# Orbiter-Finance/Plonky2-lib

Measured on AMD Instinct MI355X. Metric: proofs/sec for secp256k1 ECDSA-verify circuit; Goldilocks NTT GB/s vs HBM peak, higher is better.
Workload: dtype u64 (Goldilocks, 64-bit modular integer)

## Files before the change

### plonky2-lib_amd/csrc/circuit_create.inc

```

static int build_quotient_plan(glp_ctx *c, glp_circuit *cc) {
    const glp_circuit_desc &d = cc->d;
    std::vector<u64> desc((size_t)LIMB_GROUPS * d.num_wires * LIMB_SLOTS, 0);
    for (int g = 0; g < LIMB_GROUPS; g++) { cc->limb_jlo[g] = d.num_wires; cc->limb_jhi[g] = 0; }
    auto put = [&](u32 s, u32 col, u32 pos, u32 kl, bool flush, u32 kf, u32 ref) {
        const u32 grp = s / LIMB_SLOTS, slot = s % LIMB_SLOTS;
        desc[((size_t)grp * d.num_wires + col) * LIMB_SLOTS + slot] = 1ull | ((u64)pos << 1) | (flush ? 32ull : 0ull) | ((u64)kl << 6) | ((u64)kf << 16) | ((u64)ref << 26);
        cc->limb_jlo[grp] = std::min(cc->limb_jlo[grp], col); cc->limb_jhi[grp] = std::max(cc->limb_jhi[grp], col);
    };
    std::vector<GateShape> shape(d.num_gates);
    for (u32 gi = 0; gi < d.num_gates; gi++) gate_shape(cc->gates[gi], shape[gi]);
    std::vector<u32> limb_list;
    auto fill = [&](u32 s, u32 gi) {
        const LimbBlock &b = shape[gi].limb;
        cc->limb_gi[s] = gi;
        for (u32 i = 0; i < b.ops; i++)
            for (u32 j = 0; j < b.limbs; j++)
                put(s, b.first + b.limbs * i + j, j & 15, b.kstride * i + b.klimb + (b.descending ? b.limbs - 1 - j : j), (j & 15) == 15 || j + 1 == b.limbs,
                    b.kstride * i + b.ksum + (j >> 4), b.ref_stride * i + b.ref0 + (j >> 4));
    };
    auto limb_start = [&](u32 gi) -> u32 { return shape[gi].limb.first; };
    auto limb_weight = [&](u32 gi) -> u32 { return shape[gi].limb.limbs * shape[gi].limb.ops; };
    for (u32 gi = 0; gi < d.num_gates; gi++) {
        const glp_gate &g = cc->gates[gi];
// ... 6 lines not shown
        } else if (light && cc->light_count < 8) {
            cc->light_gi[cc->light_count++] = gi;
        } else if (g.type != GLP_GATE_NOOP) {
            cc->single_gates.push_back(gi);
        }
    }
    if (limb_list.size() == 1) {
        cc->single_gates.push_back(limb_list[0]);
        limb_list.clear();
    }
    if (!limb_list.empty()) {
        const u32 cnt = (u32)limb_list.size();
        const u32 G = (cnt + LIMB_SLOTS - 1) / LIMB_SLOTS;
        u32 used[LIMB_GROUPS] = {0, 0, 0, 0};
        std::stable_sort(limb_list.begin(), limb_list.end(), [&](u32 x, u32 y) {
            return limb_start(x) != limb_start(y) ? limb_start(x) < limb_start(y) : limb_weight(x) > limb_weight(y); });
        for (u32 t = 0; t < cnt; t++) {
            const u32 grp = t / LIMB_SLOTS;
            fill(grp * LIMB_SLOTS + used[grp], limb_list[t]);
            used[grp]++;
        }
        cc->limb_count = cnt; cc->limb_groups = G;
        for (u32 g = 0; g < G; g++) cc->limb_gcount[g] = used[g];
    }
    if (cc->limb_count) {
        std::vector<u32> keep;
        for (u32 gi : cc->single_gates) {
            if (cc->gates[gi].type == GLP_GATE_COMPARISON && cc->limb_extra_count < 4) cc->limb_extra_gi[cc->limb_extra_count++] = gi;
            else keep.push_back(gi);
        }
        cc->single_gates.swap(keep);
    }
    if (cc->limb_count) {
        GLP_TRY(c->alloc((void **)&cc->dev_limb_desc, desc.size() * 8));
        GLP_TRY(h2d(c, cc->dev_limb_desc, desc.data(), desc.size() * 8));
    }
    return GLP_OK;
}

extern "C" {

void glp_circuit_free(glp_circuit *cc) {
    if (!cc) return;
    glp_ctx *c = cc->ctx;
    (void)hipSetDevice(c->device);
    (void)hipStreamSynchronize(c->stream);
// ... 159 lines not shown
```

### plonky2-lib_amd/csrc/prover.hip

```cpp
#include <algorithm>
#include <string.h>
#include "batch.h"
#include "common.h"
#include "merkle.h"
#include "ntt.h"
#include "poseidon.h"
#include "prover_types.h"

namespace {
void make_layout(const glp_circuit_desc &c, Layout &L, bool zk) {
    const u32 cap = 1u << c.cap_height, nch = c.num_challenges;
    memset(&L, 0, sizeof(L));
    L.oracle_cols[0] = c.num_constants + c.num_routed_wires;
    L.oracle_cols[1] = c.num_wires;
    L.oracle_cols[2] = nch * (1 + c.num_partial_products);
    L.oracle_cols[3] = nch * c.quotient_degree_factor;
    for (int k = 0; k < 4; k++) L.leaf_len[k] = L.oracle_cols[k] + (zk && k > 0 ? SALT_SIZE : 0);
    L.nopen = (size_t)c.num_constants + c.num_routed_wires + c.num_wires + 2 * nch + nch * c.num_partial_products +
              nch * c.quotient_degree_factor;
    L.openings = 3 * (size_t)cap * 4;
    L.fri_caps = L.openings + 2 * L.nopen;
    L.queries = L.fri_caps + (size_t)c.num_reductions * cap * 4;
    const u32 lgN = c.degree_bits + c.rate_bits;
    L.depth0 = lgN - c.cap_height;
// ... 118 lines not shown
        GLP_TRY(commit(dev_wires, BATCH_VALUES, g.nw, wb, GLP_SALT_TAG_WIRES, 0, host_wires));
        stage = S_WIRES;
        return GLP_OK;
    }
    int partial_products(const u64 *betas_in, const u64 *gammas_in) {
        GLP_REQUIRE(stage == S_WIRES, "partial_products: call after begin");
        for (u32 i = 0; i < g.nch; i++) { betas[i] = betas_in[i]; gammas[i] = gammas_in[i]; }
        u64 *zp, *dens, *tot;
        GLP_TRY(tmp.get(&zp, (size_t)g.nzp * g.n));
        GLP_TRY(tmp.get(&dens, (size_t)g.nzp * g.n));
        GLP_TRY(tmp.get(&tot, (size_t)g.nch * nblk(g.n)));
        {
            StageScope st(c, "partial_products", 8.0 * g.n * (2.0 * g.nr + g.nzp));
            GLP_TRY(stage_partial_products(c, g, dev_wires, betas, gammas, nullptr, zp, dens, tot));
        }
        GLP_TRY(commit(zp, BATCH_VALUES, g.nzp, zb, GLP_SALT_TAG_ZS, 1));
        stage = S_ZS;
        return GLP_OK;
    }
    int quotient(const u64 *alphas) {
        GLP_REQUIRE(stage == S_ZS, "quotient: call after partial_products");
        const u32 nch = g.nch;
        const size_t apn = (size_t)nch * g.nterms, qlen = (size_t)nch * g.Rq * g.n;
        std::vector<u64> apow((1 + APL_WORDS) * apn);
        alpha_power_table(alphas, nch, g.nterms, apow.data(), apow.data() + apn);
        u64 *dev_apow, *qv, *qV, *qc;
        GLP_TRY(tmp.get(&dev_apow, apow.size()));
        GLP_TRY(h2d(c, dev_apow, apow.data(), apow.size() * 8));
        GLP_TRY(tmp.get(&qv, qlen));
        GLP_TRY(tmp.get(&qV, qlen));
        GLP_TRY(tmp.get(&qc, qlen));
        QProof qp;
        QBatch qbt;
        quotient_proof_args(g, wb.b, zb.b, qv, dev_apow, nullptr, qp, qbt);
        for (u32 i = 0; i < nch; i++) { qp.betas[i] = betas[i]; qp.gammas[i] = gammas[i]; }
        memcpy(qp.pih, pih, 32);
        {
            StageScope st(c, "quotient_eval", 8.0 * g.n * g.Rq * (g.nc + g.nr + g.nw + g.nzp + 2.0 * nch));
            u64 *l0t;
            GLP_TRY(tmp.get(&l0t, (size_t)g.Rq * g.n));
            GLP_TRY(stage_quotient_eval(c, g, qp, qbt, l0t));
        }
        {
            StageScope st(c, "quotient_intt", 16.0 * g.n * g.Rq * nch);
            GLP_TRY(stage_quotient_coeffs(c, g, qv, qV, qc));
        }
        GLP_TRY(commit(qc, BATCH_COEFFS_BITREV, nch * g.qdf, qb, GLP_SALT_TAG_QUOTIENT, 2));
        stage = S_QUOTIENT;
// ... 371 lines not shown
```

### plonky2-lib_amd/csrc/prover_batch.inc

```
#include "host_pool.h"

namespace {

int caps_to_host(glp_ctx *c, const u64 *dev_digests, size_t dig_stride_words, size_t cap_off_digests, u32 capn, u32 K, std::vector<u64> &out) {
    out.resize((size_t)K * capn * 4);
    GLP_HIP(hipMemcpy2DAsync(out.data(), (size_t)capn * 32, dev_digests + 4 * cap_off_digests, dig_stride_words * 8, (size_t)capn * 32, K,
                             hipMemcpyDeviceToHost, c->stream));
    GLP_HIP(hipStreamSynchronize(c->stream));
    return GLP_OK;
}

int prove_batch_impl(glp_ctx *c, const glp_circuit *cc, u32 K, const u64 *dev_wires, const u64 *public_inputs, u64 *proofs_out) {
    const glp_circuit_desc &d = cc->d;
    const Layout &L = cc->L;
    const ProveGeo g = prove_geo(cc, K);
    GLP_TRY(batch_check(g));
    const int lg = g.lg, rb = g.rb, hasher = g.hasher;
    const size_t n = g.n, N = g.N;
    const u32 nch = g.nch, nw = g.nw, qdf = g.qdf, nzp = g.nzp, capn = g.capn, nterms = g.nterms, npi = d.num_public_inputs;
    const u32 nred = d.num_reductions, nq = d.num_query_rounds;
    HostPool &pool = ctx_host_pool(c);
    BatchTrace mark(c, K, "");
    Tmp tmp(c);
    auto P = [&](u32 k) { return proofs_out + (size_t)k * L.total; };
// ... 16 lines not shown
    std::vector<u64> chal((size_t)K * 2 * MAXCH, 0);
    pool.run(K, [&](size_t k) {
        memcpy(P((u32)k) + L.caps, &caps[k * capn * 4], (size_t)capn * 32);
        ch[k].observe_hashes(cc->digest, 1);
        ch[k].observe(&pih[4 * k], 4);
        ch[k].observe_hashes(&caps[k * capn * 4], capn);
        for (u32 i = 0; i < nch; i++) chal[k * 2 * MAXCH + i] = ch[k].get();
        for (u32 i = 0; i < nch; i++) chal[k * 2 * MAXCH + MAXCH + i] = ch[k].get();
    });

    mark("transcript 1 (host)");
    u64 *dev_chal, *zp, *dens, *tot;
    GLP_TRY(tmp.get(&dev_chal, chal.size()));
    GLP_TRY(h2d(c, dev_chal, chal.data(), chal.size() * 8));
    GLP_TRY(tmp.get(&zp, (size_t)K * nzp * n));
    GLP_TRY(tmp.get(&dens, (size_t)K * nzp * n));
    GLP_TRY(tmp.get(&tot, (size_t)K * nch * nblk(n)));
    GLP_TRY(stage_partial_products(c, g, dev_wires, nullptr, nullptr, dev_chal, zp, dens, tot));
    GLP_TRY(batch_build(c, zp, BATCH_VALUES, nzp, lg, rb, (int)d.cap_height, &zb.b, nullptr, K, hasher, salt, GLP_SALT_TAG_ZS));
    GLP_TRY(caps_to_host(c, zb.b->digests, ndig * 4, cap_off, capn, K, caps));

    mark("partial products + commit");
    const size_t apn = (size_t)nch * nterms;
    std::vector<u64> apow((size_t)(1 + APL_WORDS) * K * apn), qpp((size_t)K * 3 * MAXCH, 0);
    pool.run(K, [&](size_t k) {
        memcpy(P((u32)k) + L.caps + capn * 4, &caps[k * capn * 4], (size_t)capn * 32);
        ch[k].observe_hashes(&caps[k * capn * 4], capn);
        u64 alphas[MAXCH];
        for (u32 i = 0; i < nch; i++) alphas[i] = ch[k].get();
        alpha_power_table(alphas, nch, nterms, &apow[k * apn], &apow[(size_t)K * apn + APL_WORDS * k * apn]);
        for (u32 i = 0; i < nch; i++) { qpp[k * 3 * MAXCH + i] = chal[k * 2 * MAXCH + i]; qpp[k * 3 * MAXCH + MAXCH + i] = chal[k * 2 * MAXCH + MAXCH + i]; }
        memcpy(&qpp[k * 3 * MAXCH + 2 * MAXCH], &pih[4 * k], 32);
    });
    mark("transcript 2 + alpha powers (host)");
    u64 *dev_apow, *dev_qpp, *qv, *qV, *qc, *l0t;
    GLP_TRY(tmp.get(&dev_apow, apow.size()));
    GLP_TRY(h2d(c, dev_apow, apow.data(), apow.size() * 8));
    GLP_TRY(tmp.get(&dev_qpp, qpp.size()));
    GLP_TRY(h2d(c, dev_qpp, qpp.data(), qpp.size() * 8));
    const size_t qstride = (size_t)nch * g.Rq * n;
    GLP_TRY(tmp.get(&qv, (size_t)K * qstride));
    GLP_TRY(tmp.get(&qV, (size_t)K * qstride));
    GLP_TRY(tmp.get(&qc, (size_t)K * qstride));
    GLP_TRY(tmp.get(&l0t, (size_t)g.Rq * n));
    {
        QProof qp;
        QBatch qbt;
        quotient_proof_args(g, wb.b, zb.b, qv, dev_apow, dev_qpp, qp, qbt);
        GLP_TRY(stage_quotient_eval(c, g, qp, qbt, l0t));
        GLP_TRY(stage_quotient_coeffs(c, g, qv, qV, qc));
    }
    GLP_TRY(batch_build(c, qc, BATCH_COEFFS_BITREV, nch * qdf, lg, rb, (int)d.cap_height, &qb.b, nullptr, K, hasher, salt, GLP_SALT_TAG_QUOTIENT));
    GLP_TRY(caps_to_host(c, qb.b->digests, ndig * 4, cap_off, capn, K, caps));
// ... 143 lines not shown
```

### plonky2-lib_amd/csrc/prover_batch_dev.inc

```
#include "transcript_dev.h"
namespace {

int prove_batch_impl_dev(glp_ctx *c, const glp_circuit *cc, u32 K, const u64 *dev_wires, const u64 *public_inputs, u64 *proofs_out) {
    const glp_circuit_desc &d = cc->d;
    const Layout &L = cc->L;
    const ProveGeo pg = prove_geo(cc, K);
    GLP_TRY(batch_check(pg));
    const int lg = pg.lg, rb = pg.rb, hasher = pg.hasher;
    const size_t n = pg.n, N = pg.N;
    const u32 nch = pg.nch, nw = pg.nw, qdf = pg.qdf, npp = pg.npp, nzp = pg.nzp, capn = pg.capn, nterms = pg.nterms, npi = d.num_public_inputs;
    const u32 nred = d.num_reductions, nq = d.num_query_rounds;
    BatchTrace mark(c, K, " dev");
    Tmp tmp(c);
    BatchHolder wb, zb, qb;
    u64 salt_seed[4] = {0, 0, 0, 0};
    const u64 *salt = nullptr;
    if (cc->zk) { GLP_TRY(salt_seed_draw(c, salt_seed)); salt = salt_seed; }
    const unsigned tgrid = (K + 15) / 16;
    u64 *dch, *image;
    u32 *dev_err;
    GLP_TRY(tmp.get(&dch, (size_t)K * DCH_WORDS));
    GLP_TRY(tmp.get(&image, (size_t)K * L.total));
    { u64 *e; GLP_TRY(tmp.get(&e, (K + 1) / 2 + 1)); dev_err = (u32 *)e; }
    GLP_HIP(hipMemsetAsync(dev_err, 0, (size_t)K * 4, c->stream));
// ... 1 lines not shown
    TrGeo g;
    g.dch = dch; g.image = image; g.total = L.total; g.K = K; g.capn = capn; g.nch = nch;

    GLP_TRY(batch_build(c, dev_wires, BATCH_VALUES, nw, lg, rb, (int)d.cap_height, &wb.b, nullptr, K, hasher, salt, GLP_SALT_TAG_WIRES));
    const size_t ndig = wb.b->ndigests, cap_off = merkle_cap_offset(N, (int)d.cap_height);
    u64 *dev_chal, *dev_qpp;
    GLP_TRY(tmp.get(&dev_chal, (size_t)K * 2 * MAXCH));
    GLP_TRY(tmp.get(&dev_qpp, (size_t)K * 3 * MAXCH));
    GLP_HIP(hipMemsetAsync(dev_chal, 0, (size_t)K * 2 * MAXCH * 8, c->stream));
    GLP_HIP(hipMemsetAsync(dev_qpp, 0, (size_t)K * 3 * MAXCH * 8, c->stream));
    hipLaunchKernelGGL(k_tr_begin, dim3(tgrid), dim3(256), 0, c->stream, g, cc->digest[0], cc->digest[1], cc->digest[2], cc->digest[3], L.pis, npi,
                       wb.b->digests + 4 * cap_off, ndig * 4, L.caps, dev_chal, dev_qpp);
    GLP_HIP(hipGetLastError());
    mark("wires commit + transcript 1");

    u64 *zp, *dens, *tot;
    GLP_TRY(tmp.get(&zp, (size_t)K * nzp * n));
    GLP_TRY(tmp.get(&dens, (size_t)K * nzp * n));
    GLP_TRY(tmp.get(&tot, (size_t)K * nch * nblk(n)));
    GLP_TRY(stage_partial_products(c, pg, dev_wires, nullptr, nullptr, dev_chal, zp, dens, tot));
    GLP_TRY(batch_build(c, zp, BATCH_VALUES, nzp, lg, rb, (int)d.cap_height, &zb.b, nullptr, K, hasher, salt, GLP_SALT_TAG_ZS));
    const size_t apn = (size_t)nch * nterms;
    u64 *dev_apow, *qv, *qV, *qc, *l0t;
    GLP_TRY(tmp.get(&dev_apow, (size_t)(1 + APL_WORDS) * K * apn));
    hipLaunchKernelGGL(k_tr_alphas, dim3(tgrid), dim3(256), 0, c->stream, g, zb.b->digests + 4 * cap_off, ndig * 4, L.caps + (size_t)capn * 4, nterms, dev_apow,
                       dev_apow + (size_t)K * apn);
    GLP_HIP(hipGetLastError());
    mark("partial products + commit + transcript 2");

    const size_t qstride = (size_t)nch * pg.Rq * n;
    GLP_TRY(tmp.get(&qv, (size_t)K * qstride));
    GLP_TRY(tmp.get(&qV, (size_t)K * qstride));
    GLP_TRY(tmp.get(&qc, (size_t)K * qstride));
    GLP_TRY(tmp.get(&l0t, (size_t)pg.Rq * n));
    {
        QProof qp;
        QBatch qbt;
        quotient_proof_args(pg, wb.b, zb.b, qv, dev_apow, dev_qpp, qp, qbt);
        GLP_TRY(stage_quotient_eval(c, pg, qp, qbt, l0t));
        GLP_TRY(stage_quotient_coeffs(c, pg, qv, qV, qc));
    }
    GLP_TRY(batch_build(c, qc, BATCH_COEFFS_BITREV, nch * qdf, lg, rb, (int)d.cap_height, &qb.b, nullptr, K, hasher, salt, GLP_SALT_TAG_QUOTIENT));
    const u64 wn = root_of_unity(lg);
    u64 *dev_zetas;
    GLP_TRY(tmp.get(&dev_zetas, (size_t)K * 4));
    hipLaunchKernelGGL(k_tr_zeta, dim3(tgrid), dim3(256), 0, c->stream, g, qb.b->digests + 4 * cap_off, ndig * 4, L.caps + 2 * (size_t)capn * 4, (u32)lg, wn, dev_zetas,
                       dev_err);
    GLP_HIP(hipGetLastError());
    mark("quotient + commit + transcript 3");
// ... 97 lines not shown
```

### plonky2-lib_amd/csrc/prover_stages.inc

```
#include <stdlib.h>
#include <chrono>

namespace {

struct ProveGeo {
    const glp_circuit *cc;
    int lg, rb, qdb, hasher, cap_height;
    size_t n, N;
    u32 nch, nr, nw, nc, qdf, npp, nzp, capn, Rq, step, nterms, K;
    const u32 *arity_bits;
    u32 nq;
};
ProveGeo prove_geo(const glp_circuit *cc, u32 K) {
    const glp_circuit_desc &d = cc->d;
    ProveGeo g;
    g.cc = cc; g.K = K;
    g.lg = (int)d.degree_bits; g.rb = (int)d.rate_bits; g.hasher = (int)d.hasher; g.cap_height = (int)d.cap_height;
    g.n = (size_t)1 << g.lg; g.N = g.n << g.rb;
    g.nch = d.num_challenges; g.nr = d.num_routed_wires; g.nw = d.num_wires; g.nc = d.num_constants;
    g.qdf = d.quotient_degree_factor; g.npp = d.num_partial_products;
    g.nzp = g.nch * (1 + g.npp); g.capn = 1u << d.cap_height;
    g.qdb = 0;
    while ((1u << g.qdb) < g.qdf) g.qdb++;
    g.Rq = 1u << g.qdb; g.step = 1u << (g.rb - g.qdb);
// ... 13 lines not shown
    for (u32 i = 0; i < MAXCH; i++) { a.betas[i] = !chal && i < nch ? betas[i] : 0; a.gammas[i] = !chal && i < nch ? gammas[i] : 0; }
    a.w_n = root_of_unity(g.lg); a.lg = lg; a.nr = g.nr; a.nch = nch; a.npp = npp; a.qdf = g.qdf;
    a.chal = chal; a.wires_stride = (size_t)g.nw * g.n; a.zp_stride = (size_t)g.nzp * g.n;
    const size_t small_lds = (size_t)2 * nch * (npp + 2) * g.n * sizeof(u64);
    if (g.lg <= 7 && small_lds <= 64 * 1024) {
        hipLaunchKernelGGL(k_pp_rows_small, dim3(1, K), dim3(256), small_lds, c->stream, a);
        GLP_HIP(hipGetLastError());
        return GLP_OK;
    }
    switch (nch) {
    case 1: hipLaunchKernelGGL(HIP_KERNEL_NAME(k_pp_rows<1>), dim3(nblocks, K), dim3(256), 0, c->stream, a); break;
    case 2: hipLaunchKernelGGL(HIP_KERNEL_NAME(k_pp_rows<2>), dim3(nblocks, K), dim3(256), 0, c->stream, a); break;
    case 3: hipLaunchKernelGGL(HIP_KERNEL_NAME(k_pp_rows<3>), dim3(nblocks, K), dim3(256), 0, c->stream, a); break;
    default: hipLaunchKernelGGL(HIP_KERNEL_NAME(k_pp_rows<4>), dim3(nblocks, K), dim3(256), 0, c->stream, a); break;
    }
    GLP_HIP(hipGetLastError());
    hipLaunchKernelGGL(k_pp_block_tot, dim3(nblocks, nch, K), dim3(256), 0, c->stream, zp, tot, lg, nblocks, a.zp_stride);
    hipLaunchKernelGGL(k_pp_scan_tot, dim3(nch, K), dim3(256), 0, c->stream, tot, nblocks);
    hipLaunchKernelGGL(k_pp_apply, dim3(nblocks, nch, K), dim3(256), 0, c->stream, zp, tot, lg, nblocks, nch, npp, a.zp_stride);
    GLP_HIP(hipGetLastError());
    return GLP_OK;
}

void alpha_power_table(const u64 *alphas, u32 nch, u32 nterms, u64 *whole, u64 *limbs) {
    for (u32 i = 0; i < nch; i++) {
        u64 x = 1;
        for (u32 t = 0; t < nterms; t++) {
            const size_t e = (size_t)i * nterms + t;
            whole[e] = x;
            apl_words(x, limbs + APL_WORDS * e);
            x = mul(x, alphas[i]);
        }
    }
}
void quotient_proof_args(const ProveGeo &g, const glp_batch *wb, const glp_batch *zb, u64 *qv, const u64 *dev_apow, const u64 *dev_pp,
                         QProof &qp, QBatch &qb) {
    memset(&qp, 0, sizeof(qp));
    qb.apow_stride = (size_t)g.nch * g.nterms;
    qp.wl = wb->lde; qp.zl = zb->lde; qp.out = qv; qp.apow = dev_apow; qp.apl = dev_apow + g.K * qb.apow_stride;
    qb.pp = dev_pp; qb.wl_stride = (size_t)(g.nw + wb->salt) * g.N; qb.zl_stride = (size_t)(g.nzp + zb->salt) * g.N;
    qb.out_stride = (size_t)g.nch * g.Rq * g.n;
}
int stage_quotient_eval(glp_ctx *c, const ProveGeo &g, const QProof &qp, const QBatch &qbt, u64 *l0t) {
    const glp_circuit *cc = g.cc;
    const glp_circuit_desc &d = cc->d;
    const u32 nch = g.nch;
    QArgs a;
    a.cs = cc->cs->lde; a.gates = cc->dev_gates; a.k_is = cc->dev_k_is; a.k_ratio = cc->k_ratio;
    const u64 WN = root_of_unity(g.lg + g.rb), gn = pow(GEN, (u64)g.n), wR = root_of_unity(g.rb);
    for (u32 rq = 0; rq < g.Rq; rq++) {
        const u32 r = rq * g.step;
        a.shift_r[rq] = mul(GEN, pow(WN, (u64)r));
        a.zh[rq] = sub(mul(gn, pow(wR, (u64)r)), 1);
        a.zh_inv[rq] = inv(a.zh[rq]);
    }
    a.w_n = root_of_unity(g.lg); a.n_field = (u64)g.n % P;
    a.lg = (u32)g.lg; a.rb = (u32)g.rb; a.step = g.step; a.nc = g.nc; a.nsel = d.num_selectors; a.nr = g.nr; a.nw = g.nw;
    a.nch = nch; a.npp = g.npp; a.qdf = g.qdf; a.num_gates = d.num_gates; a.nterms = g.nterms;
    a.many_selectors = d.num_selectors > 1;
    a.gate_mode = nch == 2 ? 1 : 0;
    a.l0 = l0t;
    hipLaunchKernelGGL(k_l0_table, dim3(nblk(g.n)), dim3(256), 0, c->stream, a, l0t, g.Rq);
    GLP_HIP(hipGetLastError());
    LightArgs lg_;
    lg_.count = cc->light_count; lg_.arith_gi = cc->arith_gi; lg_.arith_ops = cc->arith_ops;
    for (u32 i = 0; i < 8; i++) lg_.gi[i] = cc->light_gi[i];
    const dim3 grid(nblk(g.n), g.Rq, g.K);
    switch (nch) {
    case 1: hipLaunchKernelGGL(HIP_KERNEL_NAME(k_quotient<1, 1>), grid, dim3(256), 0, c->stream, a, qp, qbt, lg_); break;
    case 2:
        if (cc->light_count || cc->arith_ops) hipLaunchKernelGGL(HIP_KERNEL_NAME(k_quotient<2, 2>), grid, dim3(256), 0, c->stream, a, qp, qbt, lg_);
        else hipLaunchKernelGGL(HIP_KERNEL_NAME(k_quotient<2, 0>), grid, dim3(256), 0, c->stream, a, qp, qbt, lg_);
        break;
    case 3: hipLaunchKernelGGL(HIP_KERNEL_NAME(k_quotient<3, 1>), grid, dim3(256), 0, c->stream, a, qp, qbt, lg_); break;
    default: hipLaunchKernelGGL(HIP_KERNEL_NAME(k_quotient<4, 1>), grid, dim3(256), 0, c->stream, a, qp, qbt, lg_); break;
    }
    GLP_HIP(hipGetLastError());
    if (a.gate_mode != 1) return GLP_OK;
    if (cc->limb_count) {
        LimbArgs la;
        limb_args(cc, la);
        la.extra_count = cc->limb_extra_count;
// ... 186 lines not shown
        shift_bits += ly.ab;
        hipLaunchKernelGGL(k_fri_gather_leaf, dim3(nblk((size_t)g.nq * arity), g.K), dim3(256), 0, c->stream, ly.vals, ly.lgL, (u32)g.rb, ly.ab, dev_idx,
                           shift_bits, g.nq, dev_q + off, stride, 2 * Lsz, qsec);
        GLP_HIP(hipGetLastError());
        off += 2 * (size_t)arity;
        GLP_TRY(merkle_gather_paths(c, ly.dig, nleaves, g.cap_height, dev_idx, g.nq, dev_q + off, stride, shift_bits, g.K, ly.ndig * 4, qsec));
        off += 4 * (size_t)(ly.lgL - ly.ab - g.cap_height);
    }
    return GLP_OK;
}
int stage_queries(glp_ctx *c, const ProveGeo &g, const glp_batch *const ob[4], const std::vector<FriLayer> &layers, const u64 *dev_idx,
                  u64 *dev_q, size_t stride, size_t qsec) {
    size_t off = 0;
    for (int b = 0; b < 4; b++) GLP_TRY(queries_oracle(c, g, ob[b], b == 0, dev_idx, dev_q, stride, qsec, off));
    GLP_TRY(queries_layers(c, g, layers, dev_idx, dev_q, stride, qsec, off));
    if (off != stride) return set_error(GLP_ERR_ARG, "internal: query record layout mismatch");
    return GLP_OK;
}

int batch_check(const ProveGeo &g) {
    GLP_REQUIRE(g.nch == 2, "glp_prove_batch: num_challenges = %u (the batch path evaluates the quotient with the two-challenge kernels)", g.nch);
    GLP_REQUIRE(g.K >= 1 && g.K <= 4096, "glp_prove_batch: batch of %u proofs outside 1..4096", g.K);
    GLP_REQUIRE((size_t)g.K * g.nw * g.N * 8 <= ((size_t)64 << 30), "glp_prove_batch: batch too large (K * num_wires * 2^(degree_bits + rate_bits) words)");
    return GLP_OK;
}
struct BatchTrace {
    glp_ctx *c;
    u32 K;
    const char *tag;
    const bool on = getenv("GLP_BATCH_TRACE") != nullptr;
    std::chrono::steady_clock::time_point t_last = std::chrono::steady_clock::now();
    BatchTrace(glp_ctx *ctx, u32 K_, const char *tag_) : c(ctx), K(K_), tag(tag_) {}
    void operator()(const char *what) {
        if (!on) return;
        (void)hipStreamSynchronize(c->stream);
        const auto now = std::chrono::steady_clock::now();
        fprintf(stderr, "[glp_prove_batch K=%u%s] %-28s %8.3f ms\n", K, tag, what, std::chrono::duration<double, std::milli>(now - t_last).count());
        t_last = now;
    }
};

}
```

### plonky2-lib_amd/csrc/quotient_kernels.inc

```
__device__ __forceinline__ u64 range_product(u64 v, u32 bound) {
    if (bound == 4) {
        const u64 u = mul_nc(v, add_cnc(v, P - 3));
        return mul_nc(u, add_cnc(2, u));
    }
    u64 p = v;
    for (u32 x = 1; x + 1 < bound; x++) p = mul(p, sub(v, (u64)x));
    return bound > 1 ? mul_nc(p, sub(v, (u64)(bound - 1))) : p;
}
struct Base4Sum { u64 lo, hi; };
__device__ __forceinline__ void b4_zero(Base4Sum &b) { b.lo = 0; b.hi = 0; }
__device__ __forceinline__ void b4_add(Base4Sum &b, u64 limb, u32 j ) {
    const u32 w = 1u << (2 * j);
    b.lo += (u64)(u32)limb * w;
    b.hi += (u64)(u32)(limb >> 32) * w;
}
__device__ __forceinline__ u64 b4_value(const Base4Sum &b) {
    const u64 l = b.lo + (b.hi << 32);
    const u32 h = (u32)(b.hi >> 32) + (l < b.lo ? 1u : 0u);
    return canon(fold96_nc(l, h));
}
struct Acc160 { u32 w0, w1, w2, w3, w4; };
__device__ __forceinline__ void acc_zero(Acc160 &a) { a.w0 = a.w1 = a.w2 = a.w3 = a.w4 = 0; }
__device__ __forceinline__ void acc_fma(Acc160 &a, u64 v, u64 m) {
    const u32 v0 = (u32)v, v1 = (u32)(v >> 32), m0 = (u32)m, m1 = (u32)(m >> 32);
// ... 38 lines not shown
}
__device__ __forceinline__ u64 acc2_reduce(const AccLimb &a) {
    Acc160 w;
    acc_zero(w);
    acc_add_shifted<0>(w, a.a00); acc_add_shifted<22>(w, a.a10); acc_add_shifted<32>(w, a.a01);
    acc_add_shifted<44>(w, a.a20); acc_add_shifted<54>(w, a.a11); acc_add_shifted<76>(w, a.a21);
    return acc_reduce(w);
}

struct AccHL { u64 c0, c1, c2; };
constexpr u32 ACC3_MAX_TERMS = 512;
inline void apl_words(u64 m, u64 out[4]) {
    const u64 mp = glf::mul(m, 1ull << 32);
    out[0] = (m & 0x3FFFFFull) | (((m >> 22) & 0x3FFFFFull) << 32); out[1] = m >> 44;
    out[2] = (mp & 0x3FFFFFull) | (((mp >> 22) & 0x3FFFFFull) << 32); out[3] = mp >> 44;
}
__device__ __forceinline__ void acc3_zero(AccHL &a) { a.c0 = a.c1 = a.c2 = 0; }
__device__ __forceinline__ void acc3_fma(AccHL &a, u64 v, const u64 *ml) {
    const u32 vlo = (u32)v, vhi = (u32)(v >> 32);
    const u64 w0 = ml[0], w1 = ml[1], w2 = ml[2], w3 = ml[3];
    a.c0 += (u64)vlo * (u32)w0; a.c1 += (u64)vlo * (u32)(w0 >> 32); a.c2 += (u64)vlo * (u32)w1;
    a.c0 += (u64)vhi * (u32)w2; a.c1 += (u64)vhi * (u32)(w2 >> 32); a.c2 += (u64)vhi * (u32)w3;
}
__device__ __forceinline__ u64 acc3_reduce(const AccHL &a) {
    Acc160 w;
    acc_zero(w);
    acc_add_shifted<0>(w, a.c0); acc_add_shifted<22>(w, a.c1); acc_add_shifted<44>(w, a.c2);
    return acc_reduce(w);
}

struct QArgs {
    const u64 *cs;
    const DevGate *gates;
    const u64 *k_is;
    u64 shift_r[MAXR], zh[MAXR], zh_inv[MAXR];
    u64 w_n, n_field;
    u32 lg, rb, step, nc, nsel, nr, nw, nch, npp, qdf, num_gates, nterms, many_selectors, gate_mode;
    u32 k_ratio;
    const u64 *l0;
};
struct QProof {
    const u64 *wl, *zl;
    u64 *out;
    const u64 *apow;
    const u64 *apl;
    u64 betas[MAXCH], gammas[MAXCH], pih[4];
};
struct QBatch { const u64 *pp; size_t wl_stride, zl_stride, out_stride, apow_stride; };
static_assert(MAXCH == 4, "pp layout: 4 betas, 4 gammas, 4 words of the public-input hash");
__device__ __forceinline__ QProof q_proof(const QProof &p0, const QBatch &b) {
    QProof p = p0;
    if (b.pp) {
        const size_t k = blockIdx.z;
        p.wl += k * b.wl_stride; p.zl += k * b.zl_stride; p.out += k * b.out_stride; p.apow += k * b.apow_stride; p.apl += APL_WORDS * k * b.apow_stride;
        const u64 *q = b.pp + k * 3 * MAXCH;
        _Pragma("unroll") for (int c = 0; c < MAXCH; c++) { p.betas[c] = q[c]; p.gammas[c] = q[MAXCH + c]; p.pih[c] = q[2 * MAXCH + c]; }
    }
    return p;
}
__global__ __launch_bounds__(256) void k_l0_table(QArgs a, u64 *out, u32 Rq) {
    const size_t n = (size_t)1 << a.lg;
    const size_t q = (size_t)blockIdx.x * 256 + threadIdx.x;
    if (q >= n) return;
    const u64 wq = dpow(a.w_n, q);
    u64 d[MAXR], pre[MAXR];
    u64 run = 1;
    for (u32 rq = 0; rq < Rq; rq++) {
        d[rq] = mul(a.n_field, sub(mul(a.shift_r[rq], wq), 1));
        pre[rq] = run;
        run = mul(run, d[rq]);
    }
    u64 iv = inv(run);
    for (int rq = (int)Rq - 1; rq >= 0; rq--) {
        out[(size_t)rq * n + q] = mul(a.zh[rq], mul(iv, pre[rq]));
        iv = mul(iv, d[rq]);
    }
}
// ... 505 lines not shown
    const u32 rq = blockIdx.y, r = rq * a.step;
    const size_t slot = (size_t)r * n + q;
    u64 acc[MAXCH];
    _Pragma("unroll") for (int c = 0; c < NCH; c++) acc[c] = 0;
    const DevGate g = a.gates[gi];
    gate_contrib<NCH, TYPE>(a, p, g, N, slot, (u32)NCH + (u32)NCH * (a.npp + 1), acc);
    const size_t Rq = (size_t)gridDim.y;
    _Pragma("unroll") for (int c = 0; c < NCH; c++) {
        u64 *o = p.out + ((size_t)c * Rq + rq) * n + q;
        *o = add(*o, mul(acc[c], a.zh_inv[rq]));
    }
}

constexpr int LIMB_SLOTS = 5, LIMB_GROUPS = 4;
struct LimbArgs { const u64 *desc; u32 groups, num_wires; u32 count[LIMB_GROUPS], jlo[LIMB_GROUPS], jhi[LIMB_GROUPS]; u32 gi[LIMB_GROUPS][LIMB_SLOTS]; u32 extra_count, extra_gi[4]; };
inline void limb_args(const glp_circuit *cc, LimbArgs &la) {
    la.desc = cc->dev_limb_desc; la.groups = cc->limb_groups; la.num_wires = cc->d.num_wires;
    for (int g = 0; g < LIMB_GROUPS; g++) {
        la.count[g] = cc->limb_gcount[g]; la.jlo[g] = cc->limb_jlo[g]; la.jhi[g] = cc->limb_jhi[g];
        for (int i = 0; i < LIMB_SLOTS; i++) la.gi[g][i] = cc->limb_gi[g * LIMB_SLOTS + i];
    }
}
template <int NCH>
__global__ __launch_bounds__(256, 2) void k_quotient_limbs(QArgs a, QProof p0, QBatch qb, LimbArgs la) {
    const QProof p = q_proof(p0, qb);
    const size_t n = (size_t)1 << a.lg, N = n << a.rb;
    const size_t q = (size_t)blockIdx.x * 256 + threadIdx.x;
    if (q >= n) return;
    const u32 rq = blockIdx.y, r = rq * a.step;
    const size_t slot = (size_t)r * n + q;
    const u32 k0 = (u32)NCH + (u32)NCH * (a.npp + 1), nt = a.nterms;
    const u64 *W = p.wl + slot;
    const u64 *ap = p.apl + APL_WORDS * (size_t)k0;
    u64 acc[MAXCH];
    _Pragma("unroll") for (int c = 0; c < NCH; c++) acc[c] = 0;
#define LIMB_EMIT(S, K, V)                                                                                     \
    do {                                                                                                       \
        const u64 _v = (V);                                                                                    \
        _Pragma("unroll") for (int c2 = 0; c2 < NCH; c2++) acc3_fma(ga[S][c2], _v, ap + APL_WORDS * ((size_t)c2 * nt + (K)));   \
    } while (0)
#pragma unroll 1
    for (u32 grp = 0; grp < la.groups; grp++) {
        const u32 gcount = la.count[grp], jlo = la.jlo[grp], jhi = la.jhi[grp];
        const u64 *desc = la.desc + (size_t)grp * la.num_wires * LIMB_SLOTS;
        AccHL ga[LIMB_SLOTS][MAXCH];
        Base4Sum bs[LIMB_SLOTS];
        _Pragma("unroll") for (int s = 0; s < LIMB_SLOTS; s++) {
            b4_zero(bs[s]);
            _Pragma("unroll") for (int c = 0; c < NCH; c++) acc3_zero(ga[s][c]);
        }
        _Pragma("unroll") for (int s = 0; s < LIMB_SLOTS; s++) {
            if ((u32)s < gcount) {
                const DevGate g = a.gates[la.gi[grp][s]];
                switch (g.type) {
                case GLP_GATE_U32_ARITHMETIC: gate_terms<NCH, GLP_GATE_U32_ARITHMETIC, true>(a, p, g, N, slot, k0, ga[s]); break;
                case GLP_GATE_U32_ADD_MANY: gate_terms<NCH, GLP_GATE_U32_ADD_MANY, true>(a, p, g, N, slot, k0, ga[s]); break;
                case GLP_GATE_U32_SUBTRACTION: gate_terms<NCH, GLP_GATE_U32_SUBTRACTION, true>(a, p, g, N, slot, k0, ga[s]); break;
                default: break;
                }
            }
        }
        for (u32 j0 = jlo; j0 <= jhi; j0 += 8) {
            u64 lv[8];
            _Pragma("unroll") for (int t = 0; t < 8; t++) if (j0 + t <= jhi) lv[t] = W[(size_t)(j0 + t) * N];
            _Pragma("unroll") for (int t = 0; t < 8; t++) if (j0 + t <= jhi) {
                const u64 v = lv[t];
                const u64 *dj = desc + (size_t)(j0 + t) * LIMB_SLOTS;
                const u64 rp = range_product(v, 4);
                _Pragma("unroll") for (int s = 0; s < LIMB_SLOTS; s++) {
                    const u64 d = dj[s];
                    if (d & 1) {
                        const u32 kl = (u32)(d >> 6) & 0x3FFu;
                        _Pragma("unroll") for (int c2 = 0; c2 < NCH; c2++) acc3_fma(ga[s][c2], rp, ap + APL_WORDS * ((size_t)c2 * nt + kl));
                        b4_add(bs[s], v, (u32)(d >> 1) & 15u);
                        if (d & 32) {
                            const u32 kf = (u32)(d >> 16) & 0x3FFu, ref = (u32)(d >> 26) & 0xFFu;
                            LIMB_EMIT(s, kf, sub(b4_value(bs[s]), W[(size_t)ref * N]));
                            b4_zero(bs[s]);
                        }
                    }
                }
            }
        }
        _Pragma("unroll") for (int s = 0; s < LIMB_SLOTS; s++) {
            if ((u32)s < gcount) {
                const u64 filter = gate_filter(a, a.gates[la.gi[grp][s]], N, slot);
                _Pragma("unroll") for (int c = 0; c < NCH; c++) acc[c] = add(acc[c], mul(filter, acc3_reduce(ga[s][c])));
            }
        }
    }
#undef LIMB_EMIT
    for (u32 t = 0; t < la.extra_count; t++) {
        const DevGate g = a.gates[la.extra_gi[t]];
        if (g.type == GLP_GATE_COMPARISON) gate_contrib<NCH, GLP_GATE_COMPARISON>(a, p, g, N, slot, k0, acc);
    }
    const size_t Rq = (size_t)gridDim.y;
// ... 27 lines not shown
```

### plonky2-lib_amd/csrc/transcript_dev.h

```cpp
#pragma once
#include "poseidon.h"
#include "prover_types.h"

namespace {
__device__ __forceinline__ u64 tr_pow(u64 b, u64 e) {
    u64 r = 1;
    while (e) { if (e & 1) r = mul(r, b); b = sqr(b); e >>= 1; }
    return r;
}
constexpr u32 DCH_WORDS = 32;
struct DSponge { u64 st, inb; u32 nin, nout; };
__device__ __forceinline__ void ds_load(DSponge &s, const u64 *p, int l) {
    s.st = l < 12 ? p[l] : 0; s.inb = l < 8 ? p[12 + l] : 0; s.nin = (u32)p[28]; s.nout = (u32)p[29];
}
__device__ __forceinline__ void ds_store(const DSponge &s, u64 *p, int l, bool live) {
    if (!live) return;
    if (l < 12) p[l] = s.st;
    if (l < 8) p[12 + l] = s.inb;
    if (l == 0) { p[28] = s.nin; p[29] = s.nout; }
}
__device__ __noinline__ void ds_duplex(DSponge &s, int l, int gb) {
    if ((u32)l < s.nin) s.st = s.inb;
    s.nin = 0;
    s.st = pos::permute_coop(s.st, l, gb);
// ... 47 lines not shown
    ds_observe(s, cap, 4 * capn, l, gb);
}

__global__ __launch_bounds__(256) void k_tr_begin(TrGeo g, u64 d0, u64 d1, u64 d2, u64 d3, size_t pis_off, u32 npi, const u64 *cap_b, size_t cap_stride,
                                                  size_t caps_off, u64 *chal, u64 *qpp) {
    TR_PROLOGUE;
    u64 x = 0;
    for (u32 c0 = 0; c0 < npi; c0 += 8) {
        if (l < 8 && c0 + (u32)l < npi) x = img[pis_off + c0 + l];
        x = pos::permute_coop(x, l, gb);
    }
    const u64 pih0 = pos::shfl64(x, gb), pih1 = pos::shfl64(x, gb + 1), pih2 = pos::shfl64(x, gb + 2), pih3 = pos::shfl64(x, gb + 3);
    DSponge s;
    s.st = 0; s.inb = 0; s.nin = 0; s.nout = 0;
    ds_observe1(s, d0, l, gb); ds_observe1(s, d1, l, gb); ds_observe1(s, d2, l, gb); ds_observe1(s, d3, l, gb);
    ds_observe1(s, pih0, l, gb); ds_observe1(s, pih1, l, gb); ds_observe1(s, pih2, l, gb); ds_observe1(s, pih3, l, gb);
    tr_cap(s, cap_b + (size_t)k * cap_stride, img + caps_off, g.capn, live, l, gb);
    u64 *ck = chal + (size_t)k * 2 * MAXCH, *qk = qpp + (size_t)k * 3 * MAXCH;
    for (u32 i = 0; i < g.nch; i++) { const u64 b = ds_get(s, l, gb); if (live && l == 0) { ck[i] = b; qk[i] = b; } }
    for (u32 i = 0; i < g.nch; i++) { const u64 b = ds_get(s, l, gb); if (live && l == 0) { ck[MAXCH + i] = b; qk[MAXCH + i] = b; } }
    if (live && l == 0) { qk[2 * MAXCH] = pih0; qk[2 * MAXCH + 1] = pih1; qk[2 * MAXCH + 2] = pih2; qk[2 * MAXCH + 3] = pih3; }
    ds_store(s, dch, l, live);
}
__global__ __launch_bounds__(256) void k_tr_alphas(TrGeo g, const u64 *cap_b, size_t cap_stride, size_t caps_off, u32 nterms, u64 *apow, u64 *apl) {
    TR_PROLOGUE;
    DSponge s;
    ds_load(s, dch, l);
    tr_cap(s, cap_b + (size_t)k * cap_stride, img + caps_off, g.capn, live, l, gb);
    for (u32 i = 0; i < g.nch; i++) {
        const u64 alpha = ds_get(s, l, gb);
        u64 a16 = alpha;
#pragma unroll
        for (int j = 0; j < 4; j++) a16 = sqr(a16);
        u64 x = tr_pow(alpha, (u64)l);
        for (u32 t = (u32)l; t < nterms; t += 16) {
            const size_t e = ((size_t)k * g.nch + i) * nterms + t;
            if (live) {
                apow[e] = x;
                const u64 mp = mul(x, 1ull << 32);
                u64 *o = apl + APL_WORDS * e;
                o[0] = (x & 0x3FFFFFull) | (((x >> 22) & 0x3FFFFFull) << 32); o[1] = x >> 44;
                o[2] = (mp & 0x3FFFFFull) | (((mp >> 22) & 0x3FFFFFull) << 32); o[3] = mp >> 44;
            }
            x = mul(x, a16);
        }
    }
    ds_store(s, dch, l, live);
}
__global__ __launch_bounds__(256) void k_tr_zeta(TrGeo g, const u64 *cap_b, size_t cap_stride, size_t caps_off, u32 lg, u64 wn, u64 *zetas, u32 *err) {
    TR_PROLOGUE;
    DSponge s;
    ds_load(s, dch, l);
    tr_cap(s, cap_b + (size_t)k * cap_stride, img + caps_off, g.capn, live, l, gb);
    const ext2 zeta = ds_get_ext(s, l, gb);
    ext2 zp = zeta;
    for (u32 i = 0; i < lg; i++) zp = e_sqr(zp);
    const ext2 zn = e_scale(zeta, wn);
    if (live && l == 0) {
        u64 *z = zetas + 4 * (size_t)k;
        z[0] = zeta.a; z[1] = zeta.b; z[2] = zn.a; z[3] = zn.b;
        if (zp.a == 1 && zp.b == 0) err[k] |= 1u;
    }
    ds_store(s, dch, l, live);
}
struct OpenGeo { size_t poff[6], openings_off; u32 cols[4], nob, nch, npp, nopen; };
__global__ __launch_bounds__(256) void k_open_reduce(TrGeo g, OpenGeo og, const u64 *partial) {
    const size_t id = (size_t)blockIdx.x * 256 + threadIdx.x;
// ... 137 lines not shown
```

Measured before the change: 9.081.

## Share descending limb-run range-check sums via prefix sums with alpha-power events

Range-check terms for descending limb runs are no longer accumulated per slot with their own alpha power. Each column's range product is instead added once into a shared prefix accumulator weighted by inverse-shifted alpha powers. At each run's open and close columns the prefix sum is reduced and folded into the slot accumulator with a signed alpha power. This needs an extended alpha-power table, built on host and device, that includes negative exponents, plus validation that the indices fit. Launch bounds on the limb kernel also go from 2 to 4 blocks per SM. This trades fewer per-slot FMAs for a larger table, extra event checks and more register pressure.

```diff
diff --git a/plonky2-lib_amd/csrc/circuit_create.inc b/plonky2-lib_amd/csrc/circuit_create.inc
--- a/plonky2-lib_amd/csrc/circuit_create.inc
+++ b/plonky2-lib_amd/csrc/circuit_create.inc
@@ -52,6 +52,19 @@
         }
         cc->limb_count = cnt; cc->limb_groups = G;
         for (u32 g = 0; g < G; g++) cc->limb_gcount[g] = used[g];
+        const u32 kbase = d.num_wires - 1 + d.num_challenges + d.num_challenges * (d.num_partial_products + 1);
+        for (u32 g = 0; g < G; g++) {
+            u64 *dg = &desc[(size_t)g * d.num_wires * LIMB_SLOTS];
+            u32 terms[LIMB_SLOTS] = {};
+            const bool fits = limb_run_events(dg, LIMB_SLOTS, cc->limb_jlo[g], find_limb_runs(dg, d.num_wires, LIMB_SLOTS), kbase, terms);
+            GLP_REQUIRE(fits, "limb gates: a range-check run's alpha index exceeds the column program's field");
+            for (u32 s = 0; s < used[g]; s++) {
+                const u32 gi = cc->limb_gi[g * LIMB_SLOTS + s];
+                GLP_REQUIRE(cc->gates[gi].num_constraints - limb_weight(gi) + terms[s] <= ACC3_MAX_TERMS,
+                            "gate %u: %u accumulator terms exceed %u", gi, cc->gates[gi].num_constraints - limb_weight(gi) + terms[s], ACC3_MAX_TERMS);
+            }
+        }
+        static_assert(256 <= ACC3_MAX_TERMS, "the shared sum takes one term per wire column (num_wires <= 256 above)");
     }
     if (cc->limb_count) {
         std::vector<u32> keep;
diff --git a/plonky2-lib_amd/csrc/limb_runs.h b/plonky2-lib_amd/csrc/limb_runs.h
--- /dev/null
+++ b/plonky2-lib_amd/csrc/limb_runs.h
@@ -0,0 +1,55 @@
+#pragma once
+#include <stddef.h>
+#include <stdint.h>
+#include <vector>
+
+constexpr int LIMB_EV_CLOSE_SHIFT = 34;
+constexpr int LIMB_EV_OPEN_SHIFT = 48;
+constexpr uint64_t LIMB_EV_ANY = (1ull << LIMB_EV_CLOSE_SHIFT) | (1ull << LIMB_EV_OPEN_SHIFT);
+constexpr uint64_t LIMB_DIRECT = 1ull << 62;
+constexpr uint64_t LIMB_COL_SHARED = 1ull << 63;
+constexpr uint32_t LIMB_EV_INDEX_MAX = 0x1FFF;
+
+inline bool limb_desc_is_limb(uint64_t d) { return (d & 1) != 0; }
+inline uint32_t limb_desc_kl(uint64_t d) { return (uint32_t)(d >> 6) & 0x3FFu; }
+
+struct LimbRun { uint32_t slot, a, b; int32_t K; bool ascending; };
+inline bool limb_run_shared(const LimbRun &r) { return !r.ascending && r.b > r.a; }
+
+inline std::vector<LimbRun> find_limb_runs(const uint64_t *desc, uint32_t num_wires, uint32_t slots) {
+    std::vector<LimbRun> runs;
+    for (uint32_t s = 0; s < slots; s++) {
+        for (uint32_t a = 0; a < num_wires;) {
+            if (!limb_desc_is_limb(desc[(size_t)a * slots + s])) { a++; continue; }
+            int32_t dir = 0, k = (int32_t)limb_desc_kl(desc[(size_t)a * slots + s]);
+            uint32_t b = a;
+            while (b + 1 < num_wires && limb_desc_is_limb(desc[(size_t)(b + 1) * slots + s])) {
+                const int32_t kn = (int32_t)limb_desc_kl(desc[(size_t)(b + 1) * slots + s]), step = kn - k;
+                if ((step != 1 && step != -1) || (dir != 0 && step != dir)) break;
+                dir = step; k = kn; b++;
+            }
+            const int32_t ka = (int32_t)limb_desc_kl(desc[(size_t)a * slots + s]);
+            runs.push_back({s, a, b, dir > 0 ? ka - (int32_t)a : ka + (int32_t)a, dir > 0});
+            a = b + 1;
+        }
+    }
+    return runs;
+}
+
+inline bool limb_run_events(uint64_t *desc, uint32_t slots, uint32_t jlo, const std::vector<LimbRun> &runs, uint32_t kbase, uint32_t *terms) {
+    for (const LimbRun &r : runs) {
+        if (!limb_run_shared(r)) {
+            for (uint32_t j = r.a; j <= r.b; j++) desc[(size_t)j * slots + r.slot] |= LIMB_DIRECT;
+            terms[r.slot] += r.b - r.a + 1;
+            continue;
+        }
+        const int64_t idx = (int64_t)kbase + r.K;
+        if (idx < 0 || idx > (int64_t)LIMB_EV_INDEX_MAX) return false;
+        const uint64_t field = 1ull | ((uint64_t)idx << 1);
+        for (uint32_t j = r.a; j <= r.b; j++) desc[(size_t)j * slots] |= LIMB_COL_SHARED;
+        desc[(size_t)r.b * slots + r.slot] |= field << LIMB_EV_CLOSE_SHIFT;
+        terms[r.slot] += 1;
+        if (r.a > jlo) { desc[(size_t)(r.a - 1) * slots + r.slot] |= field << LIMB_EV_OPEN_SHIFT; terms[r.slot] += 1; }
+    }
+    return true;
+}
diff --git a/plonky2-lib_amd/csrc/prover.hip b/plonky2-lib_amd/csrc/prover.hip
--- a/plonky2-lib_amd/csrc/prover.hip
+++ b/plonky2-lib_amd/csrc/prover.hip
@@ -164,8 +164,8 @@
         GLP_REQUIRE(stage == S_ZS, "quotient: call after partial_products");
         const u32 nch = g.nch;
         const size_t apn = (size_t)nch * g.nterms, qlen = (size_t)nch * g.Rq * g.n;
-        std::vector<u64> apow((1 + APL_WORDS) * apn);
-        alpha_power_table(alphas, nch, g.nterms, apow.data(), apow.data() + apn);
+        std::vector<u64> apow(alpha_table_words(g));
+        alpha_power_table(alphas, nch, g.nterms, g.nw, apow.data(), apow.data() + apn, apow.data() + (1 + APL_WORDS) * apn);
         u64 *dev_apow, *qv, *qV, *qc;
         GLP_TRY(tmp.get(&dev_apow, apow.size()));
         GLP_TRY(h2d(c, dev_apow, apow.data(), apow.size() * 8));
diff --git a/plonky2-lib_amd/csrc/prover_batch.inc b/plonky2-lib_amd/csrc/prover_batch.inc
--- a/plonky2-lib_amd/csrc/prover_batch.inc
+++ b/plonky2-lib_amd/csrc/prover_batch.inc
@@ -62,13 +62,14 @@
 
     mark("partial products + commit");
     const size_t apn = (size_t)nch * nterms;
-    std::vector<u64> apow((size_t)(1 + APL_WORDS) * K * apn), qpp((size_t)K * 3 * MAXCH, 0);
+    const size_t apxn = apx_words(nch, nterms, nw);
+    std::vector<u64> apow((size_t)K * alpha_table_words(g)), qpp((size_t)K * 3 * MAXCH, 0);
     pool.run(K, [&](size_t k) {
         memcpy(P((u32)k) + L.caps + capn * 4, &caps[k * capn * 4], (size_t)capn * 32);
         ch[k].observe_hashes(&caps[k * capn * 4], capn);
         u64 alphas[MAXCH];
         for (u32 i = 0; i < nch; i++) alphas[i] = ch[k].get();
-        alpha_power_table(alphas, nch, nterms, &apow[k * apn], &apow[(size_t)K * apn + APL_WORDS * k * apn]);
+        alpha_power_table(alphas, nch, nterms, nw, &apow[k * apn], &apow[(size_t)K * apn + APL_WORDS * k * apn], &apow[(size_t)(1 + APL_WORDS) * K * apn + k * apxn]);
         for (u32 i = 0; i < nch; i++) { qpp[k * 3 * MAXCH + i] = chal[k * 2 * MAXCH + i]; qpp[k * 3 * MAXCH + MAXCH + i] = chal[k * 2 * MAXCH + MAXCH + i]; }
         memcpy(&qpp[k * 3 * MAXCH + 2 * MAXCH], &pih[4 * k], 32);
     });
diff --git a/plonky2-lib_amd/csrc/prover_batch_dev.inc b/plonky2-lib_amd/csrc/prover_batch_dev.inc
--- a/plonky2-lib_amd/csrc/prover_batch_dev.inc
+++ b/plonky2-lib_amd/csrc/prover_batch_dev.inc
@@ -47,9 +47,9 @@
     GLP_TRY(batch_build(c, zp, BATCH_VALUES, nzp, lg, rb, (int)d.cap_height, &zb.b, nullptr, K, hasher, salt, GLP_SALT_TAG_ZS));
     const size_t apn = (size_t)nch * nterms;
     u64 *dev_apow, *qv, *qV, *qc, *l0t;
-    GLP_TRY(tmp.get(&dev_apow, (size_t)(1 + APL_WORDS) * K * apn));
+    GLP_TRY(tmp.get(&dev_apow, (size_t)K * alpha_table_words(pg)));
     hipLaunchKernelGGL(k_tr_alphas, dim3(tgrid), dim3(256), 0, c->stream, g, zb.b->digests + 4 * cap_off, ndig * 4, L.caps + (size_t)capn * 4, nterms, dev_apow,
-                       dev_apow + (size_t)K * apn);
+                       dev_apow + (size_t)K * apn, nw, dev_apow + (size_t)(1 + APL_WORDS) * K * apn);
     GLP_HIP(hipGetLastError());
     mark("partial products + commit + transcript 2");
 
diff --git a/plonky2-lib_amd/csrc/prover_stages.inc b/plonky2-lib_amd/csrc/prover_stages.inc
--- a/plonky2-lib_amd/csrc/prover_stages.inc
+++ b/plonky2-lib_amd/csrc/prover_stages.inc
@@ -59,7 +59,10 @@
     return GLP_OK;
 }
 
-void alpha_power_table(const u64 *alphas, u32 nch, u32 nterms, u64 *whole, u64 *limbs) {
+inline u32 apx_len(u32 nterms, u32 nw) { return nterms + 2 * nw - 1; }
+inline size_t apx_words(u32 nch, u32 nterms, u32 nw) { return (size_t)2 * nch * apx_len(nterms, nw) * APL_WORDS; }
+void alpha_power_table(const u64 *alphas, u32 nch, u32 nterms, u32 nw, u64 *whole, u64 *limbs, u64 *ext) {
+    const u32 xs = apx_len(nterms, nw);
     for (u32 i = 0; i < nch; i++) {
         u64 x = 1;
         for (u32 t = 0; t < nterms; t++) {
@@ -68,13 +71,24 @@
             apl_words(x, limbs + APL_WORDS * e);
             x = mul(x, alphas[i]);
         }
-    }
+        x = pow(inv(alphas[i]), (u64)(nw - 1));
+        for (u32 t = 0; t < xs; t++) {
+            apl_words(x, ext + APL_WORDS * ((size_t)i * xs + t));
+            apl_words(neg(x), ext + APL_WORDS * ((size_t)(nch + i) * xs + t));
+            x = mul(x, alphas[i]);
+        }
+    }
+}
+inline size_t alpha_table_words(const ProveGeo &g) {
+    return (size_t)(1 + APL_WORDS) * g.nch * g.nterms + apx_words(g.nch, g.nterms, g.nw);
 }
 void quotient_proof_args(const ProveGeo &g, const glp_batch *wb, const glp_batch *zb, u64 *qv, const u64 *dev_apow, const u64 *dev_pp,
                          QProof &qp, QBatch &qb) {
     memset(&qp, 0, sizeof(qp));
     qb.apow_stride = (size_t)g.nch * g.nterms;
+    qb.apx_stride = apx_words(g.nch, g.nterms, g.nw);
     qp.wl = wb->lde; qp.zl = zb->lde; qp.out = qv; qp.apow = dev_apow; qp.apl = dev_apow + g.K * qb.apow_stride;
+    qp.apx = qp.apl + APL_WORDS * g.K * qb.apow_stride;
     qb.pp = dev_pp; qb.wl_stride = (size_t)(g.nw + wb->salt) * g.N; qb.zl_stride = (size_t)(g.nzp + zb->salt) * g.N;
     qb.out_stride = (size_t)g.nch * g.Rq * g.n;
 }
@@ -94,7 +108,7 @@
     a.w_n = root_of_unity(g.lg); a.n_field = (u64)g.n % P;
     a.lg = (u32)g.lg; a.rb = (u32)g.rb; a.step = g.step; a.nc = g.nc; a.nsel = d.num_selectors; a.nr = g.nr; a.nw = g.nw;
     a.nch = nch; a.npp = g.npp; a.qdf = g.qdf; a.num_gates = d.num_gates; a.nterms = g.nterms;
-    a.many_selectors = d.num_selectors > 1;
+    a.many_selectors = d.num_selectors > 1; a.apx_len = apx_len(g.nterms, g.nw);
     a.gate_mode = nch == 2 ? 1 : 0;
     a.l0 = l0t;
     hipLaunchKernelGGL(k_l0_table, dim3(nblk(g.n)), dim3(256), 0, c->stream, a, l0t, g.Rq);
@@ -327,6 +341,8 @@
     GLP_REQUIRE(g.nch == 2, "glp_prove_batch: num_challenges = %u (the batch path evaluates the quotient with the two-challenge kernels)", g.nch);
     GLP_REQUIRE(g.K >= 1 && g.K <= 4096, "glp_prove_batch: batch of %u proofs outside 1..4096", g.K);
     GLP_REQUIRE((size_t)g.K * g.nw * g.N * 8 <= ((size_t)64 << 30), "glp_prove_batch: batch too large (K * num_wires * 2^(degree_bits + rate_bits) words)");
+    GLP_REQUIRE((size_t)g.K * alpha_table_words(g) * 8 <= ((size_t)4 << 30), "glp_prove_batch: alpha power tables of %u proofs (%zu words each) exceed 4 GiB",
+                g.K, alpha_table_words(g));
     return GLP_OK;
 }
 struct BatchTrace {
diff --git a/plonky2-lib_amd/csrc/quotient_kernels.inc b/plonky2-lib_amd/csrc/quotient_kernels.inc
--- a/plonky2-lib_amd/csrc/quotient_kernels.inc
+++ b/plonky2-lib_amd/csrc/quotient_kernels.inc
@@ -1,3 +1,4 @@
+#include "limb_runs.h"
 __device__ __forceinline__ u64 range_product(u64 v, u32 bound) {
     if (bound == 4) {
         const u64 u = mul_nc(v, add_cnc(v, P - 3));
@@ -84,12 +85,14 @@
     a.c0 += (u64)vlo * (u32)w0; a.c1 += (u64)vlo * (u32)(w0 >> 32); a.c2 += (u64)vlo * (u32)w1;
     a.c0 += (u64)vhi * (u32)w2; a.c1 += (u64)vhi * (u32)(w2 >> 32); a.c2 += (u64)vhi * (u32)w3;
 }
-__device__ __forceinline__ u64 acc3_reduce(const AccHL &a) {
+__device__ __forceinline__ u64 acc3_reduce_nc(const AccHL &a) {
     Acc160 w;
     acc_zero(w);
     acc_add_shifted<0>(w, a.c0); acc_add_shifted<22>(w, a.c1); acc_add_shifted<44>(w, a.c2);
-    return acc_reduce(w);
-}
+    const u64 h = fold96_nc(((u64)w.w3 << 32) | w.w2, w.w4);
+    return fold128_nc(w.w0, w.w1, (u32)h, (u32)(h >> 32));
+}
+__device__ __forceinline__ u64 acc3_reduce(const AccHL &a) { return canon(acc3_reduce_nc(a)); }
 
 struct QArgs {
     const u64 *cs;
@@ -98,6 +101,7 @@
     u64 shift_r[MAXR], zh[MAXR], zh_inv[MAXR];
     u64 w_n, n_field;
     u32 lg, rb, step, nc, nsel, nr, nw, nch, npp, qdf, num_gates, nterms, many_selectors, gate_mode;
+    u32 apx_len;
     u32 k_ratio;
     const u64 *l0;
 };
@@ -106,15 +110,16 @@
     u64 *out;
     const u64 *apow;
     const u64 *apl;
+    const u64 *apx;
     u64 betas[MAXCH], gammas[MAXCH], pih[4];
 };
-struct QBatch { const u64 *pp; size_t wl_stride, zl_stride, out_stride, apow_stride; };
+struct QBatch { const u64 *pp; size_t wl_stride, zl_stride, out_stride, apow_stride, apx_stride; };
 static_assert(MAXCH == 4, "pp layout: 4 betas, 4 gammas, 4 words of the public-input hash");
 __device__ __forceinline__ QProof q_proof(const QProof &p0, const QBatch &b) {
     QProof p = p0;
     if (b.pp) {
         const size_t k = blockIdx.z;
-        p.wl += k * b.wl_stride; p.zl += k * b.zl_stride; p.out += k * b.out_stride; p.apow += k * b.apow_stride; p.apl += APL_WORDS * k * b.apow_stride;
+        p.wl += k * b.wl_stride; p.zl += k * b.zl_stride; p.out += k * b.out_stride; p.apow += k * b.apow_stride; p.apl += APL_WORDS * k * b.apow_stride; p.apx += k * b.apx_stride;
         const u64 *q = b.pp + k * 3 * MAXCH;
         _Pragma("unroll") for (int c = 0; c < MAXCH; c++) { p.betas[c] = q[c]; p.gammas[c] = q[MAXCH + c]; p.pih[c] = q[2 * MAXCH + c]; }
     }
@@ -666,7 +671,7 @@
     }
 }
 template <int NCH>
-__global__ __launch_bounds__(256, 2) void k_quotient_limbs(QArgs a, QProof p0, QBatch qb, LimbArgs la) {
+__global__ __launch_bounds__(256, 4) void k_quotient_limbs(QArgs a, QProof p0, QBatch qb, LimbArgs la) {
     const QProof p = q_proof(p0, qb);
     const size_t n = (size_t)1 << a.lg, N = n << a.rb;
     const size_t q = (size_t)blockIdx.x * 256 + threadIdx.x;
@@ -676,6 +681,8 @@
     const u32 k0 = (u32)NCH + (u32)NCH * (a.npp + 1), nt = a.nterms;
     const u64 *W = p.wl + slot;
     const u64 *ap = p.apl + APL_WORDS * (size_t)k0;
+    const u32 xs = a.apx_len, xz = la.num_wires - 1;
+    const u64 *xp = p.apx, *xn = p.apx + APL_WORDS * (size_t)NCH * xs;
     u64 acc[MAXCH];
     _Pragma("unroll") for (int c = 0; c < NCH; c++) acc[c] = 0;
 #define LIMB_EMIT(S, K, V)                                                                                     \
@@ -688,7 +695,9 @@
         const u32 gcount = la.count[grp], jlo = la.jlo[grp], jhi = la.jhi[grp];
         const u64 *desc = la.desc + (size_t)grp * la.num_wires * LIMB_SLOTS;
         AccHL ga[LIMB_SLOTS][MAXCH];
+        AccHL ps[MAXCH];
         Base4Sum bs[LIMB_SLOTS];
+        _Pragma("unroll") for (int c = 0; c < NCH; c++) acc3_zero(ps[c]);
         _Pragma("unroll") for (int s = 0; s < LIMB_SLOTS; s++) {
             b4_zero(bs[s]);
             _Pragma("unroll") for (int c = 0; c < NCH; c++) acc3_zero(ga[s][c]);
@@ -711,11 +720,30 @@
                 const u64 v = lv[t];
                 const u64 *dj = desc + (size_t)(j0 + t) * LIMB_SLOTS;
                 const u64 rp = range_product(v, 4);
+                u64 ev = 0;
+                _Pragma("unroll") for (int s = 0; s < LIMB_SLOTS; s++) ev |= dj[s];
+                if (dj[0] & LIMB_COL_SHARED) {
+                    _Pragma("unroll") for (int c2 = 0; c2 < NCH; c2++) acc3_fma(ps[c2], rp, xp + APL_WORDS * ((size_t)c2 * xs + xz - (j0 + t)));
+                }
+                if (ev & LIMB_EV_ANY) {
+                    _Pragma("unroll") for (int c2 = 0; c2 < NCH; c2++) {
+                        const u64 pv = acc3_reduce_nc(ps[c2]);
+                        _Pragma("unroll") for (int s = 0; s < LIMB_SLOTS; s++) {
+                            const u64 d = dj[s];
+                            if ((d >> LIMB_EV_CLOSE_SHIFT) & 1)
+                                acc3_fma(ga[s][c2], pv, xp + APL_WORDS * ((size_t)c2 * xs + ((u32)(d >> (LIMB_EV_CLOSE_SHIFT + 1)) & LIMB_EV_INDEX_MAX)));
+                            if ((d >> LIMB_EV_OPEN_SHIFT) & 1)
+                                acc3_fma(ga[s][c2], pv, xn + APL_WORDS * ((size_t)c2 * xs + ((u32)(d >> (LIMB_EV_OPEN_SHIFT + 1)) & LIMB_EV_INDEX_MAX)));
+                        }
+                    }
+                }
                 _Pragma("unroll") for (int s = 0; s < LIMB_SLOTS; s++) {
                     const u64 d = dj[s];
                     if (d & 1) {
-                        const u32 kl = (u32)(d >> 6) & 0x3FFu;
-                        _Pragma("unroll") for (int c2 = 0; c2 < NCH; c2++) acc3_fma(ga[s][c2], rp, ap + APL_WORDS * ((size_t)c2 * nt + kl));
+                        if (d & LIMB_DIRECT) {
+                            const u32 kl = (u32)(d >> 6) & 0x3FFu;
+                            _Pragma("unroll") for (int c2 = 0; c2 < NCH; c2++) acc3_fma(ga[s][c2], rp, ap + APL_WORDS * ((size_t)c2 * nt + kl));
+                        }
                         b4_add(bs[s], v, (u32)(d >> 1) & 15u);
                         if (d & 32) {
                             const u32 kf = (u32)(d >> 16) & 0x3FFu, ref = (u32)(d >> 26) & 0xFFu;
diff --git a/plonky2-lib_amd/csrc/transcript_dev.h b/plonky2-lib_amd/csrc/transcript_dev.h
--- a/plonky2-lib_amd/csrc/transcript_dev.h
+++ b/plonky2-lib_amd/csrc/transcript_dev.h
@@ -93,7 +93,13 @@
     if (live && l == 0) { qk[2 * MAXCH] = pih0; qk[2 * MAXCH + 1] = pih1; qk[2 * MAXCH + 2] = pih2; qk[2 * MAXCH + 3] = pih3; }
     ds_store(s, dch, l, live);
 }
-__global__ __launch_bounds__(256) void k_tr_alphas(TrGeo g, const u64 *cap_b, size_t cap_stride, size_t caps_off, u32 nterms, u64 *apow, u64 *apl) {
+__device__ __forceinline__ void tr_apl_words(u64 x, u64 *o) {
+    const u64 mp = mul(x, 1ull << 32);
+    o[0] = (x & 0x3FFFFFull) | (((x >> 22) & 0x3FFFFFull) << 32); o[1] = x >> 44;
+    o[2] = (mp & 0x3FFFFFull) | (((mp >> 22) & 0x3FFFFFull) << 32); o[3] = mp >> 44;
+}
+__global__ __launch_bounds__(256) void k_tr_alphas(TrGeo g, const u64 *cap_b, size_t cap_stride, size_t caps_off, u32 nterms, u64 *apow, u64 *apl,
+                                                   u32 nw = 0, u64 *apx = nullptr) {
     TR_PROLOGUE;
     DSponge s;
     ds_load(s, dch, l);
@@ -108,12 +114,20 @@
             const size_t e = ((size_t)k * g.nch + i) * nterms + t;
             if (live) {
                 apow[e] = x;
-                const u64 mp = mul(x, 1ull << 32);
-                u64 *o = apl + APL_WORDS * e;
-                o[0] = (x & 0x3FFFFFull) | (((x >> 22) & 0x3FFFFFull) << 32); o[1] = x >> 44;
-                o[2] = (mp & 0x3FFFFFull) | (((mp >> 22) & 0x3FFFFFull) << 32); o[3] = mp >> 44;
+                tr_apl_words(x, apl + APL_WORDS * e);
             }
             x = mul(x, a16);
+        }
+        if (apx) {
+            const u32 xs = nterms + 2 * nw - 1;
+            x = mul(tr_pow(tr_pow(alpha, P - 2), (u64)(nw - 1)), tr_pow(alpha, (u64)l));
+            for (u32 t = (u32)l; t < xs; t += 16) {
+                if (live) {
+                    tr_apl_words(x, apx + APL_WORDS * (((size_t)k * 2 * g.nch + i) * xs + t));
+                    tr_apl_words(neg(x), apx + APL_WORDS * (((size_t)k * 2 * g.nch + g.nch + i) * xs + t));
+                }
+                x = mul(x, a16);
+            }
         }
     }
     ds_store(s, dch, l, live);
```

New measurement: 8.670. 0.955x the previous value.
